# AzureLeon1/DiffSpectra

Hardware: AMD Instinct MI355X
Metric: molecules/sec, 1000-step QM9S all-spectra sampling (partial run) (higher is better)
Workload: dtype f32 (GEMMs as split-fp16 x3 MFMA with fp32 accumulate; fp32-level accuracy, parity gates unchanged)

## Files before the change

diffspectra_amd/csrc/ds_kernels.hip:

```cpp
#include <hip/hip_runtime.h>
#include <math.h>
#include <stdint.h>
#include <stdio.h>
#include <stdlib.h>

#include <atomic>
#include <mutex>
#include <utility>
#include <vector>

#include "../../include/diffspectra_hip.h"
#include "ds_device.h"
#include "ds_train_common.h"

#define ADAC DS_ADA_COLS
constexpr int DS_NODE_PF = 8;
constexpr int DS_NODE_PF2 = 4;
constexpr int DS_QKV_PF = 4;
constexpr int DS_TWO_STREAM_MAX_PAIRS = 400000;

#ifdef DS_STAMPS
#define DS_STAMP_INIT()                                                                                 \
  unsigned long long _sa[16] = {0, 0, 0, 0, 0, 0, 0, 0, 0, 0, 0, 0, 0, 0, 0, 0};                        \
  unsigned long long _t0 = __builtin_amdgcn_s_memtime()
#define DS_STAMP(i)                                                                                     \
  do {                                                                                                  \
    const unsigned long long _t1 = __builtin_amdgcn_s_memtime();                                        \
    _sa[i] += _t1 - _t0;                                                                                \
    _t0 = _t1;                                                                                          \
  } while (0)
#define DS_STAMP_W(i)                                                                                   \
  do {                                                                                                  \
    asm volatile("s_waitcnt vmcnt(0) lgkmcnt(0)" ::: "memory");                                         \
    DS_STAMP(i);                                                                                        \
  } while (0)
#define DS_STAMP_FLUSH(t)                                                                               \
  do {                                                                                                  \
    if (threadIdx.x == (t))                                                                             \
      for (int _i = 0; _i < 16; ++_i)                                                                   \
        if (_sa[_i]) atomicAdd(reinterpret_cast<unsigned long long*>(c.ws.flags + 16) + _i, _sa[_i]);   \
  } while (0)
#else
#define DS_STAMP_INIT()
#define DS_STAMP(i)
#define DS_STAMP_W(i)
#define DS_STAMP_FLUSH(t)
#endif

namespace {

struct Ctx {
  ds_layout L;
  ds_workspace ws;
  const float* wbase;
  const int64_t* woff;
  float edge_th, cutoff;
};

__device__ __forceinline__ const float* BW(const Ctx& c, int blk, int slot) {
  return c.wbase + c.woff[blk * DS_W_BLOCK_SLOTS + slot];
}
__device__ __forceinline__ const float* GW(const Ctx& c, int slot) {
  return c.wbase + c.woff[DS_NBLOCKS * DS_W_BLOCK_SLOTS + slot];
}

__device__ __forceinline__ float rbf_feature(float x, int k, const float* __restrict__ mean, const float* __restrict__ stdv,
                                             const float* __restrict__ astd) {
  if (k == 0) return x;
  const float z = (x - mean[k - 1]) / stdv[k - 1];
  return expf(-0.5f * (z * z)) / astd[k - 1];
}

// ... 175 lines not shown
  {
    const int k = kf, rb = rbp;
    const float rsk = __builtin_amdgcn_rcpf(sk), rak = __builtin_amdgcn_rcpf(ak);
    const int Pp = c.L.Pp;
#pragma unroll
    for (int j = 0; j < 16; ++j) {
      const int row = rb + 4 * j, p = row0 + row;
      const float x = xs[row];
      const float z = (x - mk) * rsk;
      float v = k ? __expf(-0.5f * (z * z)) * rak : x;
      if (p >= Pp) { v = 0.0f; ev[j] = 0.0f; }
      split_store1(&Xh[row][0], 128, k, v);
      split_store1(&Xh[row][0], 128, 64 + k, ev[j]);
    }
  }
  {
    const int wv = tid >> 6, mt = wv >> 1, cc = wv & 1, lane = tid & 63;
    const WStreamH wse = wstream_h(BW(c, blk, DS_BW_EDGE_EMB_H), 64, 128, cc * 32);
    WRingH<8> ring;
    wring_h<8>(ring, wse, 0);
    const float bcol = BW(c, blk, DS_BW_EDGE_EMB_B)[cc * 32 + (lane & 31)];
    __syncthreads();
    f32x16 acc[1], lo[1];
#pragma unroll
    for (int i = 0; i < 16; ++i) acc[0][i] = bcol;
    acc_zero<1>(lo);
    wave_mma_h_deep<1, false, 8, 8>(&Xh[mt * 32][0], 128, wse, ring, 0, acc, lo);
    split_finish<1>(acc, lo);
#pragma unroll
    for (int i = 0; i < 16; ++i) Y[mt * 32 + acc_row(i, lane >> 5)][cc * 32 + (lane & 31)] = acc[0][i];
  }
  __syncthreads();
  {
    const int lane = tid & 63, wv = tid >> 6;
    _Float16* ye = reinterpret_cast<_Float16*>(c.ws.ye);
#pragma unroll
    for (int j = 0; j < 4; ++j) {
      const int row = 16 * wv + 4 * j + (lane >> 4);
      const float4 v = ln_mod_reg64(reinterpret_cast<const float4*>(&Y[row][0])[lane & 15], lsh[j], lsc[j]);
      if (row0 + row < c.L.Pp) split_store4(ye + (size_t)(row0 + row) * 128, 64, 4 * (lane & 15), v);
    }
  }
}

template <int NW>
__global__ __launch_bounds__(NW * 64) void k_node_qkv(Ctx c, int blk) {
  ds_fp16_saturate();
  constexpr int NT = NW * 64;
  constexpr int T = 64;
  constexpr int LDH = 2 * 256 + 8;
  __shared__ __attribute__((aligned(16))) _Float16 Xh[T][LDH];
  __shared__ int rmol[T];
  const int tid = threadIdx.x, row0 = blockIdx.x * T, col0 = blockIdx.y * 384;
  if (tid < T) rmol[tid] = (row0 + tid < c.L.Nn) ? c.L.node_mol[row0 + tid] : 0;
  __syncthreads();
  {
    const float* adn = c.ws.ada + blk * DS_ADA_BLOCK_STRIDE + DS_ADA_NODE;
    const int lane = tid & 63, wv = tid >> 6, g = lane >> 4, j = lane & 15;
    static_assert(NT == 256, "four waves x 16 rows");
#pragma unroll
    for (int half = 0; half < 2; ++half) {
      float4 v[2][4], sh[2][4], sc[2][4];
#pragma unroll
      for (int ps = 0; ps < 2; ++ps) {
        const int row = 16 * wv + 8 * half + 4 * ps + g;
        const float4* hp = reinterpret_cast<const float4*>(c.ws.h + (size_t)min(row0 + row, c.L.Nn - 1) * 256) + j;
        const float4* ap = reinterpret_cast<const float4*>(adn + (size_t)rmol[row] * ADAC) + j;
#pragma unroll
        for (int u = 0; u < 4; ++u) {
          v[ps][u] = hp[16 * u];
          sh[ps][u] = ap[16 * u];
          sc[ps][u] = ap[64 + 16 * u];
        }
      }
#pragma unroll
      for (int ps = 0; ps < 2; ++ps) {
        const int row = 16 * wv + 8 * half + 4 * ps + g;
        ln_mod_quad256(v[ps], sh[ps], sc[ps]);
#pragma unroll
        for (int u = 0; u < 4; ++u)
          split_store4(&Xh[row][0], 256, 64 * u + 4 * j, row0 + row < c.L.Nn ? v[ps][u] : make_float4(0, 0, 0, 0));
      }
    }
  }
  __syncthreads();
  const float* bias = BW(c, blk, DS_BW_QKV_B) + col0;
  float* qkv = c.ws.qkv + (size_t)row0 * 768 + col0;
  const int valid = c.L.Nn - row0, wave = tid >> 6;
  for (int ch = wave; ch < 12; ch += NW) {
    asm volatile("" ::: "memory");
    const float b = bias[ch * 32 + (tid & 31)];
    f32x16 acc[2], lo[2];
#pragma unroll
    for (int m = 0; m < 2; ++m)
#pragma unroll
      for (int i = 0; i < 16; ++i) acc[m][i] = b;
    acc_zero<2>(lo);
    wave_mma_h_ring<2, false, 16, DS_QKV_PF>(&Xh[0][0], 256, BW(c, blk, DS_BW_QKV_H), 768, 256, col0 + ch * 32, 0, acc, lo);
    split_finish<2>(acc, lo);
    acc_store<2, 768>(acc, qkv + ch * 32, valid, [](int, float v) { return v; });
  }
}

__global__ __launch_bounds__(1024) void k_attn_fused(Ctx c, int blk) {
  ds_fp16_saturate();
  DS_STAMP_INIT();
  constexpr int NT = 1024, QS = 512 + 32, LDT = 256 + 4, LDY = 2 * 64 + 8, CR = 32, MAXP = DS_MAX_ATOMS * (DS_MAX_ATOMS - 1) / 2;
  __shared__ __attribute__((aligned(16))) float QK[DS_MAX_ATOMS * QS];
  __shared__ __attribute__((aligned(16))) float Tt[2][CR][LDT];
  __shared__ __attribute__((aligned(16))) _Float16 Yc[2][CR][LDY];
  __shared__ __attribute__((aligned(16))) float AL[2][CR][32];
  __shared__ int PT[(MAXP + 15) & ~15];
  __shared__ int VT[32][32];
  static_assert(DS_MAX_ATOMS <= 32 && MAXP <= 511 - CR, "visit table packing");
  static_assert(DS_MAX_ATOMS * 128 <= 4 * NT && DS_MAX_ATOMS * 64 <= 2 * NT && MAXP <= NT, "single-pass staging");
  const int tid = threadIdx.x, wave = tid >> 6, lane = tid & 63, hh = lane >> 5;
  int n0, n, p0, P;
  if (c.L.mol_by_size) {
    const int4 r = reinterpret_cast<const int4*>(c.L.mol_by_size)[blockIdx.x];
    n0 = r.x; n = r.y; p0 = r.z; P = r.w;
  } else {
    const int m = blockIdx.x;
    n0 = c.L.node_off[m]; n = c.L.node_off[m + 1] - n0;
    p0 = c.L.pair_off[m]; P = c.L.pair_off[m + 1] - p0;
  }
  const WStreamH ws_e0 = wstream_h(BW(c, blk, DS_BW_E0_H), 256, 64, (wave & 7) * 32);
  const WStreamH ws_e1 = wstream_h(BW(c, blk, DS_BW_E1_H), 256, 64, (wave & 7) * 32);
  if (n <= 0) return;
  if (P <= 0) {
    for (int i = tid; i < 256; i += NT) c.ws.attn[(size_t)n0 * 256 + i] = 0.0f;
    return;
  }
  const int nch = (P + CR - 1) / CR;
  const bool producer = wave >= 8;
  const int ptid = tid & 511, prow = ptid >> 4, ppiece = ptid & 15;
  const u32x4* ye4 = reinterpret_cast<const u32x4*>(c.ws.ye) + (size_t)p0 * 16;
  auto row_pair = [&](int R) {
    const int d = R / n + 1, i = R - (d - 1) * n;
    int j = i + d;
    if (j >= n) j -= n;
    const int a = min(i, j), b = max(i, j);
    return a * (2 * n - a - 1) / 2 + (b - a - 1);
// ... 266 lines not shown
          acc[u].x += (v[u].x * g[u].x) * al[u]; acc[u].y += (v[u].y * g[u].y) * al[u];
          acc[u].z += (v[u].z * g[u].z) * al[u]; acc[u].w += (v[u].w * g[u].w) * al[u];
        }
      }
      DS_STAMP(6);
      __syncthreads();
      DS_STAMP(7);
    };
    for (int k = 0; k < nch; k += 2) {
      interval(k, ab);
      if (k + 1 >= nch) break;
      interval(k + 1, aa);
    }
    if (t_me < n) {
      float4* o = reinterpret_cast<float4*>(c.ws.attn + (size_t)(n0 + t_me) * 256 + 4 * q16);
#pragma unroll
      for (int u = 0; u < 4; ++u) o[16 * u] = acc[u];
    }
    DS_STAMP_FLUSH(0);
  }
}

__global__ __launch_bounds__(256) void k_node_n2e(Ctx c, int blk) {
  ds_fp16_saturate();
  constexpr int T = 64, LDH = 2 * 256 + 8;
  __shared__ __attribute__((aligned(16))) _Float16 A1[T][LDH];
  const int tid = threadIdx.x, wave = tid >> 6, lane = tid & 63, row0 = blockIdx.x * T;
  const int Nn = c.L.Nn;
  {
    float4 v[16];
#pragma unroll
    for (int u = 0; u < 16; ++u) {
      const int idx = tid + u * 256, row = idx >> 6, k4 = idx & 63;
      v[u] = reinterpret_cast<const float4*>(c.ws.attn + (size_t)min(row0 + row, Nn - 1) * 256)[k4];
    }
#pragma unroll
    for (int u = 0; u < 16; ++u) {
      const int idx = tid + u * 256, row = idx >> 6, k4 = idx & 63;
      split_store4(&A1[row][0], 256, 4 * k4, row0 + row < Nn ? v[u] : make_float4(0, 0, 0, 0));
    }
  }
  __syncthreads();
  const int mt = wave >> 1, cc = wave & 1;
  if (row0 + mt * 32 >= Nn) return;
  f32x16 acc[1], lo[1];
  acc_zero<1>(acc);
  acc_zero<1>(lo);
  wave_mma_h_ring<1, false, 16, DS_NODE_PF>(&A1[mt * 32][0], 256, BW(c, blk, DS_BW_N2E_H), 64, 256, cc * 32, 0, acc, lo);
  split_finish<1>(acc, lo);
  acc_store<1, 64>(acc, c.ws.u + (size_t)(row0 + mt * 32) * 64 + cc * 32, Nn - row0 - mt * 32, [](int, float v) { return v; });
  (void)lane;
}

template <bool N2E>
__global__ __launch_bounds__(256, 2) void k_node_update(Ctx c, int blk) {
  ds_fp16_saturate();
  constexpr int T = 32, LDH = 2 * 256 + 8;
  __shared__ __attribute__((aligned(16))) _Float16 B1[T][LDH];
  __shared__ __attribute__((aligned(16))) _Float16 H2[T][LDH];
  __shared__ int rmol[T];
  const int tid = threadIdx.x, wave = tid >> 6, row0 = blockIdx.x * T;
  const int Nn = c.L.Nn;
  const float* ada = c.ws.ada;
  if (tid < T) rmol[tid] = (row0 + tid < Nn) ? c.L.node_mol[row0 + tid] : 0;
  __syncthreads();
  {
    const int lane = tid & 63, g = lane >> 4, j = lane & 15;
    float4 va[2][4], vh[2][4], vg[2][4], sh[2][4], sc[2][4];
#pragma unroll
    for (int ps = 0; ps < 2; ++ps) {
      const int row = 8 * wave + 4 * ps + g;
      const size_t gr = (size_t)min(row0 + row, Nn - 1);
      const float4* ad = reinterpret_cast<const float4*>(ada + (size_t)rmol[row] * ADAC + blk * DS_ADA_BLOCK_STRIDE + DS_ADA_NODE) + j;
      const float4* ap = reinterpret_cast<const float4*>(c.ws.attn + gr * 256) + j;
      const float4* hp = reinterpret_cast<const float4*>(c.ws.h + gr * 256) + j;
#pragma unroll
      for (int u = 0; u < 4; ++u) {
        va[ps][u] = ap[16 * u];
        vh[ps][u] = hp[16 * u];
        vg[ps][u] = ad[128 + 16 * u];
        sh[ps][u] = ad[192 + 16 * u];
        sc[ps][u] = ad[256 + 16 * u];
      }
    }
#pragma unroll
    for (int ps = 0; ps < 2; ++ps) {
      const int row = 8 * wave + 4 * ps + g;
      float4 r[4];
#pragma unroll
      for (int u = 0; u < 4; ++u) {
        if (row0 + row >= Nn) va[ps][u] = vh[ps][u] = make_float4(0, 0, 0, 0);
        if (N2E) split_store4(&B1[row][0], 256, 64 * u + 4 * j, va[ps][u]);
        r[u].x = vh[ps][u].x + vg[ps][u].x * va[ps][u].x; r[u].y = vh[ps][u].y + vg[ps][u].y * va[ps][u].y;
        r[u].z = vh[ps][u].z + vg[ps][u].z * va[ps][u].z; r[u].w = vh[ps][u].w + vg[ps][u].w * va[ps][u].w;
      }
      ln_mod_quad256(r, sh[ps], sc[ps]);
#pragma unroll
      for (int u = 0; u < 4; ++u) split_store4(&H2[row][0], 256, 64 * u + 4 * j, r[u]);
    }
  }
  __syncthreads();
  if (N2E) {
    if (wave < 2) {
      f32x16 acc[1], lo[1];
      acc_zero<1>(acc);
      acc_zero<1>(lo);
      wave_mma_h_ring<1, false, 16, DS_NODE_PF>(&B1[0][0], 256, BW(c, blk, DS_BW_N2E_H), 64, 256, wave * 32, 0, acc, lo);
      split_finish<1>(acc, lo);
      acc_store<1, 64>(acc, c.ws.u + (size_t)row0 * 64 + wave * 32, Nn - row0, [](int, float v) { return v; });
    }
    __syncthreads();
  }
  {
    const float* b1 = BW(c, blk, DS_BW_FF1_B);
    const float* W1 = BW(c, blk, DS_BW_FF1_H);
    const float* W2 = BW(c, blk, DS_BW_FF2_H);
    f32x16 acc2[2][1], lo2[2][1];
    acc_zero<1>(acc2[0]); acc_zero<1>(acc2[1]);
    acc_zero<1>(lo2[0]); acc_zero<1>(lo2[1]);
    const int mA = rmol[0], mB = rmol[min(T, Nn - row0) - 1];
    const float* gsec = ada + blk * DS_ADA_BLOCK_STRIDE + DS_ADA_NODE + 1280;
    float gAv[2], gBv[2], bbv[2];
#pragma unroll
    for (int cc = 0; cc < 2; ++cc) {
      const int col = (wave + 4 * cc) * 32 + (tid & 31);
      gAv[cc] = gsec[(size_t)mA * ADAC + col]; gBv[cc] = gsec[(size_t)mB * ADAC + col]; bbv[cc] = BW(c, blk, DS_BW_FF2_B)[col];
    }
    for (int half = 0; half < 2; ++half) {
      {
        asm volatile("" ::: "memory");
        const int hhf = (tid & 63) >> 5;
        f32x16 acc[2][1], lo[2][1];
#pragma unroll
        for (int cc = 0; cc < 2; ++cc) {
          const float bf = b1[half * 256 + (wave + 4 * cc) * 32 + (tid & 31)];
#pragma unroll
          for (int i = 0; i < 16; ++i) acc[cc][0][i] = bf;
          acc_zero<1>(lo[cc]);
        }
        wave_mma_h_ring_t2<1, false, 16, DS_NODE_PF2>(&H2[0][0], 256, wstream_h(W1, 512, 256, (half * 8 + wave) * 32),
                                                     wstream_h(W1, 512, 256, (half * 8 + wave + 4) * 32), 0, acc[0], lo[0], acc[1], lo[1]);
#pragma unroll
        for (int cc = 0; cc < 2; ++cc) {
          split_finish<1>(acc[cc], lo[cc]);
          const int colf = (wave + 4 * cc) * 32 + (tid & 31);
#pragma unroll
          for (int i = 0; i < 16; i += 2) {
            f32x2 v;
            v.x = acc[cc][0][i]; v.y = acc[cc][0][i + 1];
            v = ds_silu2(v);
            const int r0 = acc_row(i, hhf);
            split_store1(&B1[r0][0], 256, colf, v.x);
            split_store1(&B1[r0 + 1][0], 256, colf, v.y);
          }
        }
      }
      __syncthreads();
      asm volatile("" ::: "memory");
      wave_mma_h_ring_t2<1, false, 16, DS_NODE_PF2>(&B1[0][0], 256, wstream_h(W2, 256, 512, wave * 32), wstream_h(W2, 256, 512, (wave + 4) * 32),
                                                   half * 16, acc2[0], lo2[0], acc2[1], lo2[1], half * 16);
      __syncthreads();
    }
    split_finish<1>(acc2[0], lo2[0]);
    split_finish<1>(acc2[1], lo2[1]);
    const int hhl = (tid & 63) >> 5;
    const bool two = mB - mA <= 1;
    bool isB[16];
#pragma unroll
    for (int i = 0; i < 16; ++i) isB[i] = rmol[acc_row(i, hhl)] != mA;
    const int rows_here = Nn - row0;
#pragma unroll
    for (int cc = 0; cc < 2; ++cc) {
      const int col = (wave + 4 * cc) * 32 + (tid & 31);
      const float gA = gAv[cc], gB = gBv[cc], bb = bbv[cc];
      const RowStore st = row_store<256>(c.ws.h + (size_t)row0 * 256 + (wave + 4 * cc) * 32);
#pragma unroll
      for (int i = 0; i < 16; ++i) {
        const int row = acc_row(i, hhl);
        float g = isB[i] ? gB : gA;
        if (!two) { const int m = rmol[row]; if (m != mA && m != mB) g = gsec[(size_t)m * ADAC + col]; }
        const float out = split_load1(&H2[row][0], 256, col) + g * (acc2[cc][0][i] + bb);
        split_store1(&H2[row][0], 256, col, out);
        if (row < rows_here) row_put(st, ((i & 3) + 8 * (i >> 2)) * 256 * 4, out);
      }
    }
  }
  __syncthreads();
  {
    const float* br = BW(c, blk, DS_BW_NODE_RO_B);
    auto ws_of = [&](int it) {
      return it < 2 ? wstream_h(BW(c, blk, DS_BW_NODE_RO_H), 64, 256, it * 32) : wstream_h(BW(c, blk, DS_BW_AC_H), 512, 256, (it - 2) * 32);
    };
    auto bias_of = [&](int it) { return it < 2 ? br[it * 32 + (tid & 31)] : 0.0f; };
    auto store_of = [&](int it, const f32x16 (&acc)[1]) {
      if (it < 2) acc_store<1, 768>(acc, c.ws.atom_hids + (size_t)row0 * 768 + 256 + 64 * blk + it * 32, Nn - row0, [](int, float v) { return v; });
      else acc_store<1, 512>(acc, c.ws.ac + (size_t)row0 * 512 + (it - 2) * 32, Nn - row0, [](int, float v) { return v; });
    };
#pragma unroll
    for (int pr = 0; pr < 2; ++pr) {
      asm volatile("" ::: "memory");
      const int itA = wave + 8 * pr, itB = itA + 4;
      f32x16 acc[2][1], lo[2][1];
      const float bA = bias_of(itA), bB = bias_of(itB);
#pragma unroll
      for (int i = 0; i < 16; ++i) { acc[0][0][i] = bA; acc[1][0][i] = bB; }
      acc_zero<1>(lo[0]); acc_zero<1>(lo[1]);
      wave_mma_h_ring_t2<1, false, 16, DS_NODE_PF2>(&H2[0][0], 256, ws_of(itA), ws_of(itB), 0, acc[0], lo[0], acc[1], lo[1]);
      split_finish<1>(acc[0], lo[0]);
      store_of(itA, acc[0]);
      split_finish<1>(acc[1], lo[1]);
      store_of(itB, acc[1]);
    }
    if (wave < 2) {
      asm volatile("" ::: "memory");
      const int it = 16 + wave;
      f32x16 acc[1], lo[1];
      acc_zero<1>(acc);
      acc_zero<1>(lo);
      wave_mma_h_ring<1, false, 16, DS_NODE_PF>(&H2[0][0], 256, BW(c, blk, DS_BW_AC_H), 512, 256, (it - 2) * 32, 0, acc, lo);
      split_finish<1>(acc, lo);
      store_of(it, acc);
    }
  }
}

__global__ __launch_bounds__(256, 2) void k_edge_update(Ctx c, int blk) {
  ds_fp16_saturate();
  DS_STAMP_INIT();
  constexpr int R = 32, LDW = 64 + DS_LDP;
  __shared__ __attribute__((aligned(16))) float E2s[4][R][LDW];
  __shared__ __attribute__((aligned(16))) float Ds[4][R][LDW];
  __shared__ int idx_s[4][3][R];
  const int tid = threadIdx.x, wave = tid >> 6, lane = tid & 63, hh = lane >> 5, r31 = lane & 31;
  constexpr int LDW2 = 2 * 64 + 8;
  float(*E2)[LDW] = E2s[wave];
  _Float16* E2h = reinterpret_cast<_Float16*>(&E2s[wave][0][0]);
  _Float16* Dh = reinterpret_cast<_Float16*>(&Ds[wave][0][0]);
  int* rmol = idx_s[wave][0];
  int* rpa = idx_s[wave][1];
  int* rpb = idx_s[wave][2];
  const int Pp = c.L.Pp;
  const int row0 = (blockIdx.x * 4 + wave) * R;
  if (row0 >= Pp) return;
  const int valid = min(R, Pp - row0);
  const float* ada = c.ws.ada + blk * DS_ADA_BLOCK_STRIDE + DS_ADA_EDGE;
  if (lane < R) {
    const int p = min(row0 + lane, Pp - 1);
    rmol[lane] = c.L.pair_mol[p]; rpa[lane] = c.L.pair_a[p]; rpb[lane] = c.L.pair_b[p];
  }
  DS_STAMP(0);
  {
    const float4* bn = reinterpret_cast<const float4*>(BW(c, blk, DS_BW_N2E_B));
    float rm[4], rs[4], ra[4];
#pragma unroll
    for (int t = 0; t < 4; ++t) {
      const int k = 4 * (lane & 15) + t;
      rm[t] = k ? BW(c, blk, DS_BW_RBF_MEAN)[k - 1] : 0.0f;
      rs[t] = __builtin_amdgcn_rcpf(k ? BW(c, blk, DS_BW_RBF_STD)[k - 1] : 1.0f);
      ra[t] = __builtin_amdgcn_rcpf(k ? BW(c, blk, DS_BW_RBF_ASTD)[k - 1] : 1.0f);
    }
#pragma unroll
    for (int it = 0; it < 2; ++it) {
      float4 ua[4], ub[4], ve[4], vd[4], vg[4], sh[4], sc[4];
      float xd[4];
// ... 1185 lines not shown

int gemm_dispatch(const GemmArgs& g, int act, hipStream_t s) {
  if (!g.A || !g.Wp || !g.C || g.M <= 0 || g.K <= 0 || g.N <= 0 || (g.cs && !g.csh)) return DS_ERR_ARG;
  const bool big = g.M >= 512 && g.a_grp_rows <= 0 && g.c_grp_rows <= 0 && g.K % 64 == 0 && g.lda % 4 == 0 &&
                   (reinterpret_cast<uintptr_t>(g.A) & 15) == 0;
  using Kernel = void (*)(GemmArgs);
  static constexpr Kernel tile128[4] = {k_gemm_big<0>, k_gemm_big<1>, k_gemm_big<2>, k_gemm_big<3>};
  static constexpr Kernel tile64[4] = {k_gemm<0>, k_gemm<1>, k_gemm<2>, k_gemm<3>};
  if (act < 0 || act > 3) return DS_ERR_ARG;
  const int rows = big ? 128 : 64;
  hipLaunchKernelGGL(big ? tile128[act] : tile64[act], dim3((g.M + rows - 1) / rows, (g.Npad + 127) / 128), dim3(256), 0, s, g);
  return DST_CHECK_LAUNCH();
}

int gemm_simple(const float* A, int64_t lda, const float* Wp, const float* bias, float* C, int64_t ldc, int M, int K, int N,
                int act, int a_silu, hipStream_t s) {
  GemmArgs g{};
  g.A = A; g.lda = lda; g.Wp = Wp; g.bias = bias; g.C = C; g.ldc = ldc; g.M = M; g.K = K; g.N = N;
  g.Npad = (N + 31) & ~31; g.a_silu = a_silu;
  return gemm_dispatch(g, act, s);
}

enum ProfSlot { PROF_EDGE_GEOM = 0, PROF_NODE_QKV = 1, PROF_ATTN = 2, PROF_NODE_UPDATE = 3, PROF_EDGE_UPDATE = 4, PROF_EQUI_PAIRS = 5 };
struct ProfState {
  int kernel = -1;
  int every = 1;
  long long seen = 0;
  std::vector<std::pair<hipEvent_t, hipEvent_t>> pool;
  size_t used = 0;
};
ProfState g_prof;

struct ProfScope {
  hipStream_t s;
  bool on = false;
  ProfScope(int kernel, hipStream_t st) : s(st) {
    if (g_prof.kernel != kernel) return;
    if ((g_prof.seen++ % g_prof.every) != 0 || g_prof.used >= g_prof.pool.size()) return;
    on = true;
    (void)hipEventRecord(g_prof.pool[g_prof.used].first, s);
  }
  ~ProfScope() {
    if (on) (void)hipEventRecord(g_prof.pool[g_prof.used++].second, s);
  }
};

void launch_edge_geom(const Ctx& c, int blk, hipStream_t s) {
  if (c.L.Pp <= 0) return;
  ProfScope ps(PROF_EDGE_GEOM, s);
  hipLaunchKernelGGL(k_edge_geom, dim3((c.L.Pp + 63) / 64), dim3(256), 0, s, c, blk);
}
void launch_node_qkv(const Ctx& c, int blk, hipStream_t s) {
  ProfScope ps(PROF_NODE_QKV, s);
  hipLaunchKernelGGL(k_node_qkv<4>, dim3((c.L.Nn + 63) / 64, 2), dim3(256), 0, s, c, blk);
}
void launch_attn(const Ctx& c, int blk, hipStream_t s) {
  ProfScope ps(PROF_ATTN, s);
  hipLaunchKernelGGL(k_attn_fused, dim3(c.L.B), dim3(1024), 0, s, c, blk);
}
void launch_node_n2e(const Ctx& c, int blk, hipStream_t s) { hipLaunchKernelGGL(k_node_n2e, dim3((c.L.Nn + 63) / 64), dim3(256), 0, s, c, blk); }
template <bool N2E>
void launch_node_update(const Ctx& c, int blk, hipStream_t s) {
  ProfScope ps(PROF_NODE_UPDATE, s);
  hipLaunchKernelGGL(k_node_update<N2E>, dim3((c.L.Nn + 31) / 32), dim3(256), 0, s, c, blk);
}
void launch_edge_update(const Ctx& c, int blk, hipStream_t s) {
  if (c.L.Pp <= 0) return;
  ProfScope ps(PROF_EDGE_UPDATE, s);
  hipLaunchKernelGGL(k_edge_update, dim3((c.L.Pp + 127) / 128), dim3(256), 0, s, c, blk);
}
void launch_equi_pairs(const Ctx& c, int blk, hipStream_t s) {
  if (c.L.Pp <= 0) return;
  ProfScope ps(PROF_EQUI_PAIRS, s);
  hipLaunchKernelGGL(k_equi_pairs, dim3(min((c.L.Pp + 31) / 32, device_cus())), dim3((EQUI_NCW + EQUI_NLW) * 64), 0, s, c, blk);
}
void launch_pos_update(const Ctx& c, int last, hipStream_t s) { hipLaunchKernelGGL(k_pos_update, dim3(c.L.B), dim3(64), 0, s, c, last); }

}

extern "C" {

void ds_struct_sizes(int64_t* out) {
  out[0] = sizeof(ds_weights);
  out[1] = sizeof(ds_layout);
  out[2] = sizeof(ds_workspace);
  out[3] = sizeof(ds_gemm_args);
}

int ds_gemm(const ds_gemm_args* a, void* stream) {
  if (!a) return DS_ERR_ARG;
  GemmArgs g{};
  g.A = a->A; g.lda = a->lda; g.a_grp_rows = a->a_grp_rows; g.a_grp_stride = a->a_grp_stride;
  g.Wp = a->Wp; g.bias = a->bias;
  g.C = a->C; g.ldc = a->ldc; g.c_grp_rows = a->c_grp_rows; g.c_grp_stride = a->c_grp_stride;
  g.M = a->M; g.K = a->K; g.N = a->N; g.Npad = (a->N + 31) & ~31;
  g.R = a->R; g.ldr = a->ldr; g.r_grp_rows = a->r_grp_rows;
  g.cs = a->col_scale; g.csh = a->col_shift; g.a_silu = a->a_silu;
  return gemm_dispatch(g, a->act, (hipStream_t)stream);
}

int ds_gemm_split(const void* A_split, const float* W_split, const float* bias, float* C, int64_t ldc, int32_t M, int32_t K,
                  int32_t N, void* stream) {
  if (!A_split || !W_split || !C || M <= 0 || K <= 0 || N <= 0 || K % 64 != 0 || N % 32 != 0 || ldc < N) return DS_ERR_ARG;
  hipLaunchKernelGGL(k_gemm_ada, dim3((M + 63) / 64, (N + 127) / 128), dim3(256), 0, (hipStream_t)stream,
                     reinterpret_cast<const _Float16*>(A_split), W_split, bias, C, (int)ldc, M, K, N);
  return DST_CHECK_LAUNCH();
}

int ds_stage_time(const ds_weights* w, const ds_layout* L, ds_workspace* ws, const float* noise_level, const float* ctx_emb,
                  void* stream) {
  hipStream_t s = (hipStream_t)stream;
  Ctx c;
  if (!make_ctx(c, w, L, ws) || !noise_level) return DS_ERR_ARG;
  const int B = L->B;
  const int64_t* off = w->off + DS_NBLOCKS * DS_W_BLOCK_SLOTS;
  hipLaunchKernelGGL(k_time_feat, dim3((B + 63) / 64), dim3(64), 0, s, c, noise_level);
  int st = gemm_simple(ws->tfeat, 24, w->base + off[DS_GW_TM1_W], w->base + off[DS_GW_TM1_B], ws->tmid, 1024, B, 24, 1024, 2, 0, s);
  if (st) return st;
  float* tm3 = ws->ada;
  st = gemm_simple(ws->tmid, 1024, w->base + off[DS_GW_TM3_W], w->base + off[DS_GW_TM3_B], tm3, 1024, B, 1024, 1024, 0, 0, s);
  if (st) return st;
  const size_t tot = (size_t)B * 1024;
  hipLaunchKernelGGL(k_temb_finish, dim3((unsigned)((tot + 255) / 256)), dim3(256), 0, s, c, (const float*)tm3, B, ctx_emb);
  static_assert(ADAC % 32 == 0, "adaLN table width");
  return ds_gemm_split(ws->temb_silu, w->base + off[DS_GW_ADA_W], w->base + off[DS_GW_ADA_B], ws->ada, ADAC, B, 1024, ADAC, stream);
}

int ds_stage_init(const ds_weights* w, const ds_layout* L, ds_workspace* ws, const float* xh, const float* edge_x,
                  const float* cond_x, const float* cond_edge_x, void* stream) {
  hipStream_t s = (hipStream_t)stream;
  Ctx c;
  if (!make_ctx(c, w, L, ws) || !xh || !edge_x || ((cond_x == nullptr) != (cond_edge_x == nullptr))) return DS_ERR_ARG;
  if (!clear(ws->flags, 8 * sizeof(int32_t), s)) return DS_ERR_LAUNCH;
  if (L->Pp > 0) hipLaunchKernelGGL(k_pair_flags, dim3((L->Pp + 1023) / 1024), dim3(1024), 0, s, c, cond_x, cond_edge_x);
  hipLaunchKernelGGL(k_node_init, dim3((L->Nn + 7) / 8), dim3(256), 0, s, c, xh, cond_x);
  if (L->Pp > 0) hipLaunchKernelGGL(k_pair_init, dim3((L->Pp + 63) / 64), dim3(256), 0, s, c, edge_x, cond_x, cond_edge_x);
  return DST_CHECK_LAUNCH();
}

int ds_stage_block(const ds_weights* w, const ds_layout* L, ds_workspace* ws, int blk, int last, void* stream) {
  hipStream_t s = (hipStream_t)stream;
  Ctx c;
  if (!make_ctx(c, w, L, ws) || blk < 0 || blk >= DS_NBLOCKS) return DS_ERR_ARG;
  launch_edge_geom(c, blk, s);
  launch_node_qkv(c, blk, s);
  launch_attn(c, blk, s);
  launch_node_update<true>(c, blk, s);
  launch_edge_update(c, blk, s);
  launch_equi_pairs(c, blk, s);
  launch_pos_update(c, last, s);
  return DST_CHECK_LAUNCH();
}

int ds_stage_readout(const ds_weights* w, const ds_layout* L, ds_workspace* ws, float* out_xh, float* out_edge, void* stream) {
  hipStream_t s = (hipStream_t)stream;
  Ctx c;
  if (!make_ctx(c, w, L, ws) || !out_xh || !out_edge) return DS_ERR_ARG;
  const size_t nx = (size_t)L->B * L->N * 9, ne = (size_t)L->B * L->N * L->N * 2;
  if (!clear(out_xh, nx * sizeof(float), s) || !clear(out_edge, ne * sizeof(float), s)) return DS_ERR_LAUNCH;
  hipLaunchKernelGGL(k_node_readout, dim3((L->Nn + 31) / 32), dim3(256), 0, s, c, out_xh);
  if (L->Pp > 0) hipLaunchKernelGGL(k_edge_readout, dim3((L->Pp + 127) / 128), dim3(256), 0, s, c, out_edge);
  hipLaunchKernelGGL(k_final_pos, dim3((L->B + 63) / 64), dim3(64), 0, s, c, out_xh);
  return DST_CHECK_LAUNCH();
}

struct SideStream {
  hipStream_t s = nullptr;
  hipEvent_t fork[DS_NBLOCKS + 1] = {}, join[DS_NBLOCKS + 1] = {};
  std::once_flag once;
  bool ok = false;
};
static SideStream g_side[MAX_DEVICES];
static int g_two_stream = -1;

static SideStream* side_stream() {
  int dev = 0;
  if (hipGetDevice(&dev) != hipSuccess || dev < 0 || dev >= MAX_DEVICES) return nullptr;
  SideStream& ss = g_side[dev];
  std::call_once(ss.once, [&ss] {
    bool ok = hipStreamCreateWithFlags(&ss.s, hipStreamNonBlocking) == hipSuccess;
    for (int i = 0; ok && i <= DS_NBLOCKS; ++i)
      ok = hipEventCreateWithFlags(&ss.fork[i], hipEventDisableTiming) == hipSuccess &&
           hipEventCreateWithFlags(&ss.join[i], hipEventDisableTiming) == hipSuccess;
    ss.ok = ok;
  });
  return ss.ok ? &ss : nullptr;
}

static int forward_blocks_two_streams(const ds_weights* w, const ds_layout* L, ds_workspace* ws, hipStream_t s, SideStream* ss) {
  Ctx c;
  if (!make_ctx(c, w, L, ws)) return DS_ERR_ARG;
  hipStream_t s2 = ss->s;
  const hipEvent_t fork0 = ss->fork[DS_NBLOCKS], join0 = ss->join[DS_NBLOCKS];
  if (!record(fork0, s) || !wait(s2, fork0)) return DS_ERR_LAUNCH;
  launch_node_qkv(c, 0, s2);
  if (!record(join0, s2)) return DS_ERR_LAUNCH;
  for (int blk = 0; blk < DS_NBLOCKS; ++blk) {
    launch_edge_geom(c, blk, s);
    if (!wait(s, blk == 0 ? join0 : ss->join[blk - 1])) return DS_ERR_LAUNCH;
    launch_attn(c, blk, s);
    launch_node_n2e(c, blk, s);
    if (!record(ss->fork[blk], s) || !wait(s2, ss->fork[blk])) return DS_ERR_LAUNCH;
    launch_node_update<false>(c, blk, s2);
    if (blk + 1 < DS_NBLOCKS) launch_node_qkv(c, blk + 1, s2);
    if (!record(ss->join[blk], s2)) return DS_ERR_LAUNCH;
    launch_edge_update(c, blk, s);
    if (!wait(s, ss->join[blk])) return DS_ERR_LAUNCH;
    launch_equi_pairs(c, blk, s);
    launch_pos_update(c, blk == DS_NBLOCKS - 1 ? 1 : 0, s);
  }
  return DST_CHECK_LAUNCH();
}

int ds_set_two_stream(int on) {
  const int prev = g_two_stream;
  g_two_stream = on;
  return prev;
}

int ds_forward(const ds_weights* w, const ds_layout* L, ds_workspace* ws, const float* xh, const float* edge_x,
               const float* cond_x, const float* cond_edge_x, const float* noise_level, const float* ctx_emb, float* out_xh,
               float* out_edge, void* stream) {
  int st = ds_stage_time(w, L, ws, noise_level, ctx_emb, stream);
  if (st) return st;
  st = ds_stage_init(w, L, ws, xh, edge_x, cond_x, cond_edge_x, stream);
  if (st) return st;
  static const int env_two = [] { const char* e = getenv("DIFFSPECTRA_TWO_STREAM"); return e ? atoi(e) : -1; }();
  const int pick = g_two_stream >= 0 ? g_two_stream : env_two;
  const int two = pick >= 0 ? pick : (L->Pp < DS_TWO_STREAM_MAX_PAIRS ? 1 : 0);
  SideStream* ss = two ? side_stream() : nullptr;
  if (ss) {
    st = forward_blocks_two_streams(w, L, ws, (hipStream_t)stream, ss);
    if (st) return st;
  } else {
    for (int b = 0; b < DS_NBLOCKS; ++b) {
      st = ds_stage_block(w, L, ws, b, b == DS_NBLOCKS - 1, stream);
      if (st) return st;
    }
  }
  return ds_stage_readout(w, L, ws, out_xh, out_edge, stream);
}

int ds_sampler_step(const ds_layout* L, float c_x, float c_pred, float sigma, float temperature, float* x, float* edge_x,
                     const float* pred, const float* edge_pred, const float* raw_pos, const float* raw_feat,
                     const float* raw_edge, float* x_mean, float* edge_mean, void* stream) {
  if (!layout_ok(L) || !x || !edge_x || !pred || !edge_pred || !raw_pos || !raw_feat || !raw_edge || !x_mean || !edge_mean) return DS_ERR_ARG;
  hipLaunchKernelGGL(k_sampler_step, dim3(L->B), dim3(256), 0, (hipStream_t)stream, *L, c_x, c_pred, sigma, temperature, x,
                     edge_x, pred, edge_pred, raw_pos, raw_feat, raw_edge, x_mean, edge_mean);
  return DST_CHECK_LAUNCH();
}

int ds_initial_noise(const ds_layout* L, uint64_t seed, const int64_t* mol_id, float* x, float* edge_x, void* stream) {
  if (!layout_ok(L) || !mol_id || !x || !edge_x) return DS_ERR_ARG;
  hipStream_t s = (hipStream_t)stream;
  const size_t nb = (size_t)L->B * L->N;
  if (!clear(x, nb * 9 * sizeof(float), s) || !clear(edge_x, nb * L->N * 2 * sizeof(float), s)) return DS_ERR_LAUNCH;
  hipLaunchKernelGGL(k_noise_step<0>, dim3(L->B), dim3(256), 0, s, *L, 0.0f, 0.0f, 0.0f, 0.0f, (unsigned long long)seed, 0u, mol_id,
                     x, edge_x, (const float*)nullptr, (const float*)nullptr, (float*)nullptr, (float*)nullptr,
                     (const float*)nullptr, (const int32_t*)nullptr);
  return DST_CHECK_LAUNCH();
}

int ds_sampler_step_philox(const ds_layout* L, float c_x, float c_pred, float sigma, float temperature, uint64_t seed, int32_t step,
                           const int64_t* mol_id, float* x, float* edge_x, const float* pred, const float* edge_pred,
                           float* x_mean, float* edge_mean, void* stream) {
  if (!layout_ok(L) || !mol_id || !x || !edge_x || !pred || !edge_pred || !x_mean || !edge_mean || step < 0) return DS_ERR_ARG;
  hipLaunchKernelGGL(k_noise_step<1>, dim3(L->B), dim3(256), 0, (hipStream_t)stream, *L, c_x, c_pred, sigma, temperature,
                     (unsigned long long)seed, (unsigned int)step + 1u, mol_id, x, edge_x, pred, edge_pred, x_mean, edge_mean,
                     (const float*)nullptr, (const int32_t*)nullptr);
  return DST_CHECK_LAUNCH();
}

int ds_step_begin(const float* table, int32_t n_steps, int32_t* step, int32_t B, float* noise_level, void* stream) {
  if (!table || !step || !noise_level || B <= 0 || n_steps <= 0) return DS_ERR_ARG;
  hipLaunchKernelGGL(k_step_begin, dim3(1), dim3(256), 0, (hipStream_t)stream, table, n_steps, step, B, noise_level);
  return DST_CHECK_LAUNCH();
}

int ds_sampler_step_philox_dev(const ds_layout* L, const float* table, const int32_t* step, float temperature, uint64_t seed,
                               const int64_t* mol_id, float* x, float* edge_x, const float* pred, const float* edge_pred,
                               float* x_mean, float* edge_mean, void* stream) {
  if (!layout_ok(L) || !table || !step || !mol_id || !x || !edge_x || !pred || !edge_pred || !x_mean || !edge_mean) return DS_ERR_ARG;
  hipLaunchKernelGGL(k_noise_step<2>, dim3(L->B), dim3(256), 0, (hipStream_t)stream, *L, 0.0f, 0.0f, 0.0f, temperature,
                     (unsigned long long)seed, 0u, mol_id, x, edge_x, pred, edge_pred, x_mean, edge_mean, table, step);
  return DST_CHECK_LAUNCH();
// ... 69 lines not shown
```

include/diffspectra_hip.h:

```cpp
#ifndef DIFFSPECTRA_HIP_H
#define DIFFSPECTRA_HIP_H

#include <stdint.h>

#ifdef __cplusplus
extern "C" {
#endif

#define DS_OK 0
#define DS_ERR_ARG (-1)
#define DS_ERR_LAUNCH (-2)

#define DS_NBLOCKS 8
#define DS_HID 256
#define DS_EHID 64
#define DS_TDIM 1024
#define DS_ADA_BLOCK_STRIDE 2464
#define DS_ADA_NODE 0
#define DS_ADA_EDGE 1536
#define DS_ADA_EQUI 1920
#define DS_ADA_DIST 2432
#define DS_ADA_TOP (DS_NBLOCKS * DS_ADA_BLOCK_STRIDE)
#define DS_ADA_COLS (DS_ADA_TOP + 32)

// ... 70 lines not shown
  const int32_t* node_dense;
  const int32_t* node_mol;
  const int32_t* pair_a;
  const int32_t* pair_b;
  const int32_t* pair_mol;
  const int32_t* mol_by_size;
} ds_layout;

typedef struct ds_workspace {
  float* pos;
  float* h;
  float* e;
  float* atom_hids;
  float* edge_hids;
  float* tfeat;
  float* tmid;
  float* temb_silu;
  float* ada;
  float* qkv;
  float* ye;
  float* dist;
  float* attn;
  float* u;
  float* ac;
  float* ed;
  float* lg;
  float* tr;
  int32_t* adj;
  int32_t* flags;
} ds_workspace;

void ds_struct_sizes(int64_t* out);

typedef struct ds_gemm_args {
  const float* A; int64_t lda; int32_t a_grp_rows; int32_t _p0; int64_t a_grp_stride;
  const float* Wp; const float* bias;
  float* C; int64_t ldc; int32_t c_grp_rows; int32_t _p1; int64_t c_grp_stride;
  int32_t M, K, N, act;
  const float* R; int64_t ldr; int32_t r_grp_rows; int32_t a_silu;
  const float* col_scale; const float* col_shift;
} ds_gemm_args;
int ds_gemm(const ds_gemm_args* args, void* stream);

int ds_gemm_split(const void* A_split, const float* W_split, const float* bias, float* C, int64_t ldc, int32_t M, int32_t K,
                  int32_t N, void* stream);

int ds_forward(const ds_weights* w, const ds_layout* L, ds_workspace* ws,
               const float* xh, const float* edge_x, const float* cond_x, const float* cond_edge_x,
               const float* noise_level, const float* ctx_emb,
               float* out_xh, float* out_edge, void* stream);

int ds_set_two_stream(int on);

int ds_stage_time(const ds_weights* w, const ds_layout* L, ds_workspace* ws, const float* noise_level,
                  const float* ctx_emb, void* stream);
int ds_stage_init(const ds_weights* w, const ds_layout* L, ds_workspace* ws, const float* xh, const float* edge_x,
                  const float* cond_x, const float* cond_edge_x, void* stream);
int ds_stage_block(const ds_weights* w, const ds_layout* L, ds_workspace* ws, int block, int last, void* stream);
int ds_stage_readout(const ds_weights* w, const ds_layout* L, ds_workspace* ws, float* out_xh, float* out_edge,
                     void* stream);

int ds_sampler_step(const ds_layout* L, float c_x, float c_pred, float sigma, float temperature,
                    float* x, float* edge_x, const float* pred, const float* edge_pred,
                    const float* raw_pos, const float* raw_feat, const float* raw_edge,
                    float* x_mean, float* edge_mean, void* stream);

int ds_initial_noise(const ds_layout* L, uint64_t seed, const int64_t* mol_id, float* x, float* edge_x, void* stream);
int ds_sampler_step_philox(const ds_layout* L, float c_x, float c_pred, float sigma, float temperature,
                           uint64_t seed, int32_t step, const int64_t* mol_id,
                           float* x, float* edge_x, const float* pred, const float* edge_pred,
                           float* x_mean, float* edge_mean, void* stream);

int ds_step_begin(const float* table, int32_t n_steps, int32_t* step, int32_t B, float* noise_level, void* stream);
int ds_sampler_step_philox_dev(const ds_layout* L, const float* table, const int32_t* step, float temperature,
                               uint64_t seed, const int64_t* mol_id, float* x, float* edge_x, const float* pred,
                               const float* edge_pred, float* x_mean, float* edge_mean, void* stream);

int ds_post_process(const ds_layout* L, const float* xh, const float* edge_x,
                    float* pos_out, int32_t* atom_type, int32_t* fc, float* edge_type, void* stream);

int ds_check_stability(const ds_layout* L, const float* pos, const int32_t* atom_type, int32_t* bond_order,
                       int32_t* nr_stable, int32_t* mol_stable, void* stream);

int ds_match_records(const uint8_t* prb_rec, const int32_t* prb_n, int64_t P, const uint8_t* ref_rec, const int32_t* ref_n, int64_t M,
                     const int64_t* ref_index, float max_distance, int32_t min_atoms, double* rmsd, int32_t* n_matched,
                     float* type_acc, float* bond_acc, uint8_t* exact, int32_t* map, void* stream);

#define DS_GRAPH_DIFFERENT 0
#define DS_GRAPH_IDENTICAL 1
#define DS_GRAPH_UNDECIDED 2
#define DS_GRAPH_INVALID 3
#define DS_GRAPH_MAX_NODES 1048576
int ds_graph_identity_records(const uint8_t* prb_rec, const int32_t* prb_n, int64_t P, const uint8_t* ref_rec, const int32_t* ref_n, int64_t M,
                              const int64_t* ref_index, int32_t max_nodes, uint8_t* verdict, int32_t* nodes, int32_t* map, void* stream);

int ds_graph_hash_records(const uint8_t* rec, const int32_t* n, int64_t P, uint64_t* hash, void* stream);

#define DS_MCES_EXACT 0
#define DS_MCES_UNDECIDED 2
#define DS_MCES_INVALID 3
#define DS_MCES_MAX_NODES 4194304
int ds_mces_records(const uint8_t* prb_rec, const int32_t* prb_n, int64_t P, const uint8_t* ref_rec, const int32_t* ref_n, int64_t M,
                    const int64_t* ref_index, int32_t drop_h, int32_t max_nodes, int32_t* dist, int32_t* lower, uint8_t* status,
                    int32_t* nodes, int32_t* map, void* stream);

#define DS_MORGAN_MAX_RADIUS 3
// ... 48 lines not shown
```

Measured before the change: 237.6.

## Fuse next block's node QKV projection into node update kernel

```diff
diff --git a/diffspectra_amd/csrc/ds_kernels.hip b/diffspectra_amd/csrc/ds_kernels.hip
--- a/diffspectra_amd/csrc/ds_kernels.hip
+++ b/diffspectra_amd/csrc/ds_kernels.hip
@@ -18,6 +18,7 @@
 constexpr int DS_NODE_PF2 = 4;
 constexpr int DS_QKV_PF = 4;
 constexpr int DS_TWO_STREAM_MAX_PAIRS = 400000;
+constexpr int DS_NODE_FUSION_MAX_PAIRS = 1000000;
 
 #ifdef DS_STAMPS
 #define DS_STAMP_INIT()                                                                                 \
@@ -299,6 +300,7 @@
   __shared__ __attribute__((aligned(16))) _Float16 Xh[T][LDH];
   __shared__ int rmol[T];
   const int tid = threadIdx.x, row0 = blockIdx.x * T, col0 = blockIdx.y * 384;
+  const int nch = gridDim.y == 1 ? 24 : 12;
   if (tid < T) rmol[tid] = (row0 + tid < c.L.Nn) ? c.L.node_mol[row0 + tid] : 0;
   __syncthreads();
   {
@@ -334,7 +336,7 @@
   const float* bias = BW(c, blk, DS_BW_QKV_B) + col0;
   float* qkv = c.ws.qkv + (size_t)row0 * 768 + col0;
   const int valid = c.L.Nn - row0, wave = tid >> 6;
-  for (int ch = wave; ch < 12; ch += NW) {
+  for (int ch = wave; ch < nch; ch += NW) {
     asm volatile("" ::: "memory");
     const float b = bias[ch * 32 + (tid & 31)];
     f32x16 acc[2], lo[2];
@@ -707,7 +709,7 @@
   (void)lane;
 }
 
-template <bool N2E>
+template <bool N2E, bool QKV>
 __global__ __launch_bounds__(256, 2) void k_node_update(Ctx c, int blk) {
   ds_fp16_saturate();
   constexpr int T = 32, LDH = 2 * 256 + 8;
@@ -717,6 +719,10 @@
   const int tid = threadIdx.x, wave = tid >> 6, row0 = blockIdx.x * T;
   const int Nn = c.L.Nn;
   const float* ada = c.ws.ada;
+  constexpr int LDF = 256 + 4;
+  static_assert(LDF * sizeof(float) == LDH * sizeof(_Float16), "the fp32 tile aliases B1 row by row");
+  float* HF = reinterpret_cast<float*>(&B1[0][0]);
+  float4 qsh[2][4], qsc[2][4];
   if (tid < T) rmol[tid] = (row0 + tid < Nn) ? c.L.node_mol[row0 + tid] : 0;
   __syncthreads();
   {
@@ -818,6 +824,15 @@
     }
     split_finish<1>(acc2[0], lo2[0]);
     split_finish<1>(acc2[1], lo2[1]);
+    if (QKV) {
+      const int lane = tid & 63, g = lane >> 4, j = lane & 15;
+#pragma unroll
+      for (int ps = 0; ps < 2; ++ps) {
+        const float4* ap = reinterpret_cast<const float4*>(ada + (size_t)rmol[8 * wave + 4 * ps + g] * ADAC + (blk + 1) * DS_ADA_BLOCK_STRIDE + DS_ADA_NODE) + j;
+#pragma unroll
+        for (int u = 0; u < 4; ++u) { qsh[ps][u] = ap[16 * u]; qsc[ps][u] = ap[64 + 16 * u]; }
+      }
+    }
     const int hhl = (tid & 63) >> 5;
     const bool two = mB - mA <= 1;
     bool isB[16];
@@ -836,11 +851,28 @@
         if (!two) { const int m = rmol[row]; if (m != mA && m != mB) g = gsec[(size_t)m * ADAC + col]; }
         const float out = split_load1(&H2[row][0], 256, col) + g * (acc2[cc][0][i] + bb);
         split_store1(&H2[row][0], 256, col, out);
+        if (QKV) HF[row * LDF + col] = out;
         if (row < rows_here) row_put(st, ((i & 3) + 8 * (i >> 2)) * 256 * 4, out);
       }
     }
   }
   __syncthreads();
+  if (QKV) {
+    const int lane = tid & 63, g = lane >> 4, j = lane & 15;
+    float4 v[2][4];
+#pragma unroll
+    for (int ps = 0; ps < 2; ++ps)
+#pragma unroll
+      for (int u = 0; u < 4; ++u) v[ps][u] = reinterpret_cast<const float4*>(HF + (8 * wave + 4 * ps + g) * LDF)[j + 16 * u];
+    __builtin_amdgcn_fence(__ATOMIC_ACQ_REL, "workgroup");
+    __builtin_amdgcn_wave_barrier();
+#pragma unroll
+    for (int ps = 0; ps < 2; ++ps) {
+      ln_mod_quad256(v[ps], qsh[ps], qsc[ps]);
+#pragma unroll
+      for (int u = 0; u < 4; ++u) split_store4(&B1[8 * wave + 4 * ps + g][0], 256, 64 * u + 4 * j, v[ps][u]);
+    }
+  }
   {
     const float* br = BW(c, blk, DS_BW_NODE_RO_B);
     auto ws_of = [&](int it) {
@@ -865,6 +897,28 @@
       store_of(itA, acc[0]);
       split_finish<1>(acc[1], lo[1]);
       store_of(itB, acc[1]);
+    }
+    if (QKV) {
+      const float* bq = BW(c, blk + 1, DS_BW_QKV_B);
+      const float* Wq = BW(c, blk + 1, DS_BW_QKV_H);
+      float* qkv = c.ws.qkv + (size_t)row0 * 768;
+      __syncthreads();
+#pragma unroll 1
+      for (int pr = 0; pr < 3; ++pr) {
+        asm volatile("" ::: "memory");
+        const int chA = wave + 8 * pr, chB = chA + 4;
+        f32x16 acc[2][1], lo[2][1];
+        const float bA = bq[chA * 32 + (tid & 31)], bB = bq[chB * 32 + (tid & 31)];
+#pragma unroll
+        for (int i = 0; i < 16; ++i) { acc[0][0][i] = bA; acc[1][0][i] = bB; }
+        acc_zero<1>(lo[0]); acc_zero<1>(lo[1]);
+        wave_mma_h_ring_t2<1, false, 16, DS_NODE_PF2>(&B1[0][0], 256, wstream_h(Wq, 768, 256, chA * 32), wstream_h(Wq, 768, 256, chB * 32), 0,
+                                                     acc[0], lo[0], acc[1], lo[1]);
+        split_finish<1>(acc[0], lo[0]);
+        acc_store<1, 768>(acc[0], qkv + chA * 32, Nn - row0, [](int, float v) { return v; });
+        split_finish<1>(acc[1], lo[1]);
+        acc_store<1, 768>(acc[1], qkv + chB * 32, Nn - row0, [](int, float v) { return v; });
+      }
     }
     if (wave < 2) {
       asm volatile("" ::: "memory");
@@ -2156,7 +2210,8 @@
 }
 void launch_node_qkv(const Ctx& c, int blk, hipStream_t s) {
   ProfScope ps(PROF_NODE_QKV, s);
-  hipLaunchKernelGGL(k_node_qkv<4>, dim3((c.L.Nn + 63) / 64, 2), dim3(256), 0, s, c, blk);
+  const int tiles = (c.L.Nn + 63) / 64;
+  hipLaunchKernelGGL(k_node_qkv<4>, dim3(tiles, tiles >= 4 * device_cus() ? 1 : 2), dim3(256), 0, s, c, blk);
 }
 void launch_attn(const Ctx& c, int blk, hipStream_t s) {
   ProfScope ps(PROF_ATTN, s);
@@ -2164,9 +2219,10 @@
 }
 void launch_node_n2e(const Ctx& c, int blk, hipStream_t s) { hipLaunchKernelGGL(k_node_n2e, dim3((c.L.Nn + 63) / 64), dim3(256), 0, s, c, blk); }
 template <bool N2E>
-void launch_node_update(const Ctx& c, int blk, hipStream_t s) {
+void launch_node_update(const Ctx& c, int blk, bool qkv, hipStream_t s) {
   ProfScope ps(PROF_NODE_UPDATE, s);
-  hipLaunchKernelGGL(k_node_update<N2E>, dim3((c.L.Nn + 31) / 32), dim3(256), 0, s, c, blk);
+  if (qkv) hipLaunchKernelGGL((k_node_update<N2E, true>), dim3((c.L.Nn + 31) / 32), dim3(256), 0, s, c, blk);
+  else hipLaunchKernelGGL((k_node_update<N2E, false>), dim3((c.L.Nn + 31) / 32), dim3(256), 0, s, c, blk);
 }
 void launch_edge_update(const Ctx& c, int blk, hipStream_t s) {
   if (c.L.Pp <= 0) return;
@@ -2249,10 +2305,25 @@
   launch_edge_geom(c, blk, s);
   launch_node_qkv(c, blk, s);
   launch_attn(c, blk, s);
-  launch_node_update<true>(c, blk, s);
+  launch_node_update<true>(c, blk, false, s);
   launch_edge_update(c, blk, s);
   launch_equi_pairs(c, blk, s);
   launch_pos_update(c, last, s);
+  return DST_CHECK_LAUNCH();
+}
+
+static int forward_blocks_fused(const ds_weights* w, const ds_layout* L, ds_workspace* ws, hipStream_t s) {
+  Ctx c;
+  if (!make_ctx(c, w, L, ws)) return DS_ERR_ARG;
+  launch_node_qkv(c, 0, s);
+  for (int blk = 0; blk < DS_NBLOCKS; ++blk) {
+    launch_edge_geom(c, blk, s);
+    launch_attn(c, blk, s);
+    launch_node_update<true>(c, blk, blk + 1 < DS_NBLOCKS, s);
+    launch_edge_update(c, blk, s);
+    launch_equi_pairs(c, blk, s);
+    launch_pos_update(c, blk == DS_NBLOCKS - 1 ? 1 : 0, s);
+  }
   return DST_CHECK_LAUNCH();
 }
 
@@ -2276,6 +2347,7 @@
 };
 static SideStream g_side[MAX_DEVICES];
 static int g_two_stream = -1;
+static int g_node_fusion = -1;
 
 static SideStream* side_stream() {
   int dev = 0;
@@ -2291,7 +2363,7 @@
   return ss.ok ? &ss : nullptr;
 }
 
-static int forward_blocks_two_streams(const ds_weights* w, const ds_layout* L, ds_workspace* ws, hipStream_t s, SideStream* ss) {
+static int forward_blocks_two_streams(const ds_weights* w, const ds_layout* L, ds_workspace* ws, hipStream_t s, SideStream* ss, bool fused) {
   Ctx c;
   if (!make_ctx(c, w, L, ws)) return DS_ERR_ARG;
   hipStream_t s2 = ss->s;
@@ -2305,8 +2377,8 @@
     launch_attn(c, blk, s);
     launch_node_n2e(c, blk, s);
     if (!record(ss->fork[blk], s) || !wait(s2, ss->fork[blk])) return DS_ERR_LAUNCH;
-    launch_node_update<false>(c, blk, s2);
-    if (blk + 1 < DS_NBLOCKS) launch_node_qkv(c, blk + 1, s2);
+    launch_node_update<false>(c, blk, fused && blk + 1 < DS_NBLOCKS, s2);
+    if (!fused && blk + 1 < DS_NBLOCKS) launch_node_qkv(c, blk + 1, s2);
     if (!record(ss->join[blk], s2)) return DS_ERR_LAUNCH;
     launch_edge_update(c, blk, s);
     if (!wait(s, ss->join[blk])) return DS_ERR_LAUNCH;
@@ -2319,6 +2391,12 @@
 int ds_set_two_stream(int on) {
   const int prev = g_two_stream;
   g_two_stream = on;
+  return prev;
+}
+
+int ds_set_node_fusion(int on) {
+  const int prev = g_node_fusion;
+  g_node_fusion = on;
   return prev;
 }
 
@@ -2332,9 +2410,15 @@
   static const int env_two = [] { const char* e = getenv("DIFFSPECTRA_TWO_STREAM"); return e ? atoi(e) : -1; }();
   const int pick = g_two_stream >= 0 ? g_two_stream : env_two;
   const int two = pick >= 0 ? pick : (L->Pp < DS_TWO_STREAM_MAX_PAIRS ? 1 : 0);
+  static const int env_fus = [] { const char* e = getenv("DIFFSPECTRA_NODE_FUSION"); return e ? atoi(e) : -1; }();
+  const int pickf = g_node_fusion >= 0 ? g_node_fusion : env_fus;
+  const bool fused = pickf >= 0 ? pickf != 0 : L->Pp < DS_NODE_FUSION_MAX_PAIRS;
   SideStream* ss = two ? side_stream() : nullptr;
   if (ss) {
-    st = forward_blocks_two_streams(w, L, ws, (hipStream_t)stream, ss);
+    st = forward_blocks_two_streams(w, L, ws, (hipStream_t)stream, ss, fused);
+    if (st) return st;
+  } else if (fused) {
+    st = forward_blocks_fused(w, L, ws, (hipStream_t)stream);
     if (st) return st;
   } else {
     for (int b = 0; b < DS_NBLOCKS; ++b) {
diff --git a/include/diffspectra_hip.h b/include/diffspectra_hip.h
--- a/include/diffspectra_hip.h
+++ b/include/diffspectra_hip.h
@@ -146,6 +146,8 @@
 
 int ds_set_two_stream(int on);
 
+int ds_set_node_fusion(int on);
+
 int ds_stage_time(const ds_weights* w, const ds_layout* L, ds_workspace* ws, const float* noise_level,
                   const float* ctx_emb, void* stream);
 int ds_stage_init(const ds_weights* w, const ds_layout* L, ds_workspace* ws, const float* xh, const float* edge_x,
```

New measurement: 239.5, median of 6. No clear change (+0.8%).
